# Xjh-UCAS/TAM-TR

Measured on AMD Instinct MI355X. Metric: images/sec fwd+bwd @640x640 bs=16/GPU, higher is better.
Workload: dtype bf16

## Files before the change

tam-tr_amd/csrc/dwconv.hip:

```cpp
#include "common.h"

namespace {

constexpr int TS = 16;
constexpr int DW_THREADS = TS * TS;
#ifndef DW_CB_BWD
#define DW_CB_BWD 16
#endif
constexpr int CB_FWD = 32, CB_BWD = DW_CB_BWD;

__device__ __forceinline__ float silu_f(float v) { return v / (1.f + __expf(-v)); }

template <typename T>
struct Vec16;
template <>
struct Vec16<float> {
  static constexpr int N = 4;
  static __device__ __forceinline__ void ld(const float* p, float (&o)[4]) {
    const float4 v = *reinterpret_cast<const float4*>(p);
    o[0] = v.x; o[1] = v.y; o[2] = v.z; o[3] = v.w;
  }
  static __device__ __forceinline__ void st(float* p, const float (&v)[4]) { *reinterpret_cast<float4*>(p) = make_float4(v[0], v[1], v[2], v[3]); }
};
template <>
struct Vec16<bf16_t> {
  static constexpr int N = 8;
  static __device__ __forceinline__ void ld(const bf16_t* p, float (&o)[8]) {
    const uint4 v = *reinterpret_cast<const uint4*>(p);
    const uint32_t w[4] = {v.x, v.y, v.z, v.w};
#pragma unroll
    for (int i = 0; i < 4; ++i) { o[2 * i] = __uint_as_float(w[i] << 16); o[2 * i + 1] = __uint_as_float(w[i] & 0xffff0000u); }
  }
  static __device__ __forceinline__ void st(bf16_t* p, const float (&v)[8]) {
    uint4 o;
    o.x = (uint32_t)f2bf(v[0]) | ((uint32_t)f2bf(v[1]) << 16); o.y = (uint32_t)f2bf(v[2]) | ((uint32_t)f2bf(v[3]) << 16);
    o.z = (uint32_t)f2bf(v[4]) | ((uint32_t)f2bf(v[5]) << 16); o.w = (uint32_t)f2bf(v[6]) | ((uint32_t)f2bf(v[7]) << 16);
    *reinterpret_cast<uint4*>(p) = o;
  }
};

__device__ __forceinline__ void plane_st(float* p, float v) { *p = v; }
__device__ __forceinline__ void plane_st(bf16_t* p, float v) { *p = f2bf(v); }
__device__ __forceinline__ float plane_ld(const float* p) { return *p; }
__device__ __forceinline__ float plane_ld(const bf16_t* p) { return bf2f(*p); }
__device__ __forceinline__ float4 plane_ld4(const float* p) { return *reinterpret_cast<const float4*>(p); }
__device__ __forceinline__ float4 plane_ld4(const bf16_t* p) {
  const uint2 v = *reinterpret_cast<const uint2*>(p);
  return make_float4(__uint_as_float(v.x << 16), __uint_as_float(v.x & 0xffff0000u), __uint_as_float(v.y << 16), __uint_as_float(v.y & 0xffff0000u));
}

template <typename T, int CB, int HALO, int PITCH>
__device__ __forceinline__ void stage_tile(const T* __restrict__ x, size_t xs, int b, int d0, int h0, int w0, int H, int W,
                                           float (*s)[TS + 2 * HALO][PITCH]) {
  constexpr int SIDE = TS + 2 * HALO, VN = Vec16<T>::N, GROUPS = CB / VN, TOTAL = SIDE * SIDE * GROUPS;
  constexpr int N_IT = (TOTAL + DW_THREADS - 1) / DW_THREADS;
  float v[N_IT][VN];
#pragma unroll
  for (int k = 0; k < N_IT; ++k) {
    const int it = min((int)threadIdx.x + k * DW_THREADS, TOTAL - 1);
    const int pix = it / GROUPS, gq = it - pix * GROUPS;
    const int py = pix / SIDE, px = pix - py * SIDE;
    const int h = min(max(h0 + py - HALO, 0), H - 1), w = min(max(w0 + px - HALO, 0), W - 1);
    Vec16<T>::ld(x + ((size_t)(b * H + h) * W + w) * xs + d0 + gq * VN, v[k]);
  }
#pragma unroll
  for (int k = 0; k < N_IT; ++k) {
    const int it = threadIdx.x + k * DW_THREADS;
    if (it < TOTAL) {
      const int pix = it / GROUPS, gq = it - pix * GROUPS;
      const int py = pix / SIDE, px = pix - py * SIDE;
      const int h = h0 + py - HALO, w = w0 + px - HALO;
      const float keep = (h >= 0 && h < H && w >= 0 && w < W) ? 1.f : 0.f;
#pragma unroll
      for (int j = 0; j < VN; ++j) s[gq * VN + j][py][px] = v[k][j] * keep;
    }
  }
}

template <typename T, typename PT>
__global__ __launch_bounds__(DW_THREADS) void dwconv_cross_fwd_kernel(const T* __restrict__ x, size_t xs, const float* __restrict__ wgt,
                                                                       const float* __restrict__ bias, PT* __restrict__ u2, int D,
                                                                       int H, int W, int tiles_w) {
  constexpr int CB = CB_FWD, SIDE = TS + 2, PITCH = SIDE + 1;
  __shared__ float s_in[CB][SIDE][PITCH];
  __shared__ float s_w[CB][10];
  const int th = blockIdx.x / tiles_w, tw = blockIdx.x - th * tiles_w;
  const int d0 = blockIdx.y * CB, b = blockIdx.z, h0 = th * TS, w0 = tw * TS;
  const size_t L = (size_t)H * W;
  for (int i = threadIdx.x; i < CB * 10; i += DW_THREADS) {
    const int c = i / 10, k = i - c * 10;
    s_w[c][k] = k < 9 ? wgt[(size_t)(d0 + c) * 9 + k] : (bias ? bias[d0 + c] : 0.f);
  }
  stage_tile<T, CB, 1, PITCH>(x, xs, b, d0, h0, w0, H, W, s_in);
  __syncthreads();
#pragma unroll
  for (int pass = 0; pass < 2; ++pass) {
    const int ty = pass == 0 ? threadIdx.x / TS : threadIdx.x % TS;
    const int tx = pass == 0 ? threadIdx.x % TS : threadIdx.x / TS;
    const int h = h0 + ty, w = w0 + tx;
    if (h >= H || w >= W) continue;
    PT* out = u2 + ((size_t)(b * 2 + pass) * D + d0) * L + (pass == 0 ? (size_t)h * W + w : (size_t)w * H + h);
    for (int c = 0; c < CB; ++c) {
      float acc = s_w[c][9];
#pragma unroll
      for (int ky = 0; ky < 3; ++ky)
#pragma unroll
        for (int kx = 0; kx < 3; ++kx) acc = fmaf(s_w[c][ky * 3 + kx], s_in[c][ty + ky][tx + kx], acc);
      plane_st(out + (size_t)c * L, silu_f(acc));
    }
  }
}

template <typename T, typename PT>
__global__ __launch_bounds__(DW_THREADS) void dwconv_cross_bwd_kernel(const PT* __restrict__ g2, const T* __restrict__ x, size_t xs,
                                                                       const float* __restrict__ wgt, const float* __restrict__ bias,
                                                                       T* __restrict__ gx, size_t gxs, float* __restrict__ ws, int D,
                                                                       int H, int W, int tiles_w, int tiles) {
  constexpr int CB = CB_BWD, XS = TS + 4, XP = XS + 1, GS = TS + 2, GP = GS + 1;
  __shared__ float s_x[CB][XS][XP];
  __shared__ float s_g[CB][GS][GP];
  __shared__ float s_w[CB][10];
  const int th = blockIdx.x / tiles_w, tw = blockIdx.x - th * tiles_w;
  const int d0 = blockIdx.y * CB, b = blockIdx.z, h0 = th * TS, w0 = tw * TS;
  const size_t L = (size_t)H * W;
  for (int i = threadIdx.x; i < CB * 10; i += DW_THREADS) {
    const int c = i / 10, k = i - c * 10;
    s_w[c][k] = k < 9 ? wgt[(size_t)(d0 + c) * 9 + k] : (bias ? bias[d0 + c] : 0.f);
  }
#ifndef DW_ABL_NOX
  stage_tile<T, CB, 2, XP>(x, xs, b, d0, h0, w0, H, W, s_x);
#endif
#ifndef DW_ABL_NOG
  if ((W & 3) == 0 && (H & 3) == 0) {
    constexpr int NV = 6, ITEMS_V = CB * GS * NV, N_ITV = (ITEMS_V + DW_THREADS - 1) / DW_THREADS;
#pragma unroll
    for (int plane = 0; plane < 2; ++plane) {
      const PT* gp = g2 + ((size_t)(b * 2 + plane) * D + d0) * L;
      float4 v[N_ITV];
#pragma unroll
      for (int k = 0; k < N_ITV; ++k) {
        const int it = min((int)threadIdx.x + k * DW_THREADS, ITEMS_V - 1);
        const int c = it / (GS * NV), r = it - c * (GS * NV), line = r / NV, q = r - line * NV;
        const int fixed = (plane == 0 ? h0 : w0) + line - 1, base = (plane == 0 ? w0 : h0) - 4 + 4 * q;
        const int nfix = plane == 0 ? H : W, nrun = plane == 0 ? W : H;
        const bool ok = fixed >= 0 && fixed < nfix && base >= 0 && base + 3 < nrun;
        const float4 t = plane_ld4(gp + (size_t)c * L + (size_t)min(max(fixed, 0), nfix - 1) * nrun + min(max(base, 0), nrun - 4));
        const float f = ok ? 1.f : 0.f;
        v[k] = make_float4(t.x * f, t.y * f, t.z * f, t.w * f);
      }
      if (plane == 1) __syncthreads();
#pragma unroll
      for (int k = 0; k < N_ITV; ++k) {
        const int it = threadIdx.x + k * DW_THREADS;
        if (it < ITEMS_V) {
          const int c = it / (GS * NV), r = it - c * (GS * NV), line = r / NV, q = r - line * NV;
          const float e[4] = {v[k].x, v[k].y, v[k].z, v[k].w};
#pragma unroll
          for (int j = 0; j < 4; ++j) {
            const int pos = 4 * q + j - 3;
            if (pos >= 0 && pos < GS) {
              if (plane == 0) s_g[c][line][pos] = e[j];
              else s_g[c][pos][line] += e[j];
            }
          }
        }
      }
    }
  } else {
  {
    constexpr int GB = 7, N_IT = ((CB * GS * GS + DW_THREADS - 1) / DW_THREADS + GB - 1) / GB * GB;
    const PT* gp = g2 + ((size_t)(b * 2 + 0) * D + d0) * L;
#pragma unroll 1
    for (int k0 = 0; k0 < N_IT; k0 += GB) {
      float v[GB];
#pragma unroll
      for (int k = 0; k < GB; ++k) {
        const int it = min((int)threadIdx.x + (k0 + k) * DW_THREADS, CB * GS * GS - 1);
        const int c = it / (GS * GS), r = it - c * (GS * GS), py = r / GS, px = r - py * GS;
        const int h = h0 + py - 1, w = w0 + px - 1;
        const bool ok = h >= 0 && h < H && w >= 0 && w < W;
        v[k] = plane_ld(gp + (size_t)c * L + (size_t)min(max(h, 0), H - 1) * W + min(max(w, 0), W - 1)) * (ok ? 1.f : 0.f);
      }
#pragma unroll
      for (int k = 0; k < GB; ++k) {
        const int it = threadIdx.x + (k0 + k) * DW_THREADS;
        if (it < CB * GS * GS) {
          const int c = it / (GS * GS), r = it - c * (GS * GS), py = r / GS, px = r - py * GS;
          s_g[c][py][px] = v[k];
        }
      }
    }
  }
  __syncthreads();
  {
    constexpr int GB = 7, N_IT = ((CB * GS * GS + DW_THREADS - 1) / DW_THREADS + GB - 1) / GB * GB;
    const PT* gp = g2 + ((size_t)(b * 2 + 1) * D + d0) * L;
#pragma unroll 1
    for (int k0 = 0; k0 < N_IT; k0 += GB) {
      float v[GB];
#pragma unroll
      for (int k = 0; k < GB; ++k) {
        const int it = min((int)threadIdx.x + (k0 + k) * DW_THREADS, CB * GS * GS - 1);
        const int c = it / (GS * GS), r = it - c * (GS * GS), px = r / GS, py = r - px * GS;
        const int h = h0 + py - 1, w = w0 + px - 1;
        const bool ok = h >= 0 && h < H && w >= 0 && w < W;
        v[k] = plane_ld(gp + (size_t)c * L + (size_t)min(max(w, 0), W - 1) * H + min(max(h, 0), H - 1)) * (ok ? 1.f : 0.f);
      }
#pragma unroll
      for (int k = 0; k < GB; ++k) {
        const int it = threadIdx.x + (k0 + k) * DW_THREADS;
        if (it < CB * GS * GS) {
          const int c = it / (GS * GS), r = it - c * (GS * GS), px = r / GS, py = r - px * GS;
          s_g[c][py][px] += v[k];
        }
      }
    }
  }
  }
#endif
  __syncthreads();
#ifndef DW_ABL_NOSILU
  {
    constexpr int TPC = DW_THREADS / CB;
    static_assert(DW_THREADS % CB == 0 && TPC <= WAVE && (TPC & (TPC - 1)) == 0, "a power-of-two lane group per channel");
    const int c = threadIdx.x / TPC, sub = threadIdx.x % TPC;
    float wk[9], dwk[10];
#pragma unroll
    for (int k9 = 0; k9 < 9; ++k9) { wk[k9] = s_w[c][k9]; dwk[k9] = 0.f; }
    dwk[9] = 0.f;
    const float bc = s_w[c][9];
    for (int r = sub; r < GS * GS; r += TPC) {
      const int px = r / GS, py = r - px * GS;
      const int h = h0 + py - 1, w = w0 + px - 1;
      float g = 0.f;
      if (h >= 0 && h < H && w >= 0 && w < W) {
        g = s_g[c][py][px];
        float xin[9], acc = bc;
#pragma unroll
        for (int ky = 0; ky < 3; ++ky)
#pragma unroll
          for (int kx = 0; kx < 3; ++kx) { xin[ky * 3 + kx] = s_x[c][py + ky][px + kx]; acc = fmaf(wk[ky * 3 + kx], xin[ky * 3 + kx], acc); }
        const float sg = 1.f / (1.f + __expf(-acc));
        g *= sg * (1.f + acc * (1.f - sg));
        if (py >= 1 && py <= TS && px >= 1 && px <= TS) {
#pragma unroll
          for (int k9 = 0; k9 < 9; ++k9) dwk[k9] = fmaf(g, xin[k9], dwk[k9]);
          dwk[9] += g;
        }
      }
      s_g[c][py][px] = g;
    }
#pragma unroll
    for (int k9 = 0; k9 < 10; ++k9) dwk[k9] = group_sum<TPC>(dwk[k9]);
    if (sub == 0) {
      float* o = ws + (((size_t)b * tiles + blockIdx.x) * D + d0 + c) * 10;
#pragma unroll
      for (int k9 = 0; k9 < 10; ++k9) o[k9] = dwk[k9];
    }
  }
#endif
  __syncthreads();
  const int ty = threadIdx.x / TS, tx = threadIdx.x % TS;
  float dxv[CB];
#pragma unroll
  for (int c = 0; c < CB; ++c) {
    float acc = 0.f;
#pragma unroll
    for (int ky = 0; ky < 3; ++ky)
#pragma unroll
      for (int kx = 0; kx < 3; ++kx) acc = fmaf(s_w[c][ky * 3 + kx], s_g[c][ty + 2 - ky][tx + 2 - kx], acc);
    dxv[c] = acc;
  }
  __syncthreads();
#pragma unroll
  for (int c = 0; c < CB; ++c) s_x[c][ty][tx] = dxv[c];
  __syncthreads();
  constexpr int VN = Vec16<T>::N, GROUPS = CB / VN;
  for (int it = threadIdx.x; it < TS * TS * GROUPS; it += DW_THREADS) {
    const int pix = it / GROUPS, gq = it - pix * GROUPS, py = pix / TS, px = pix - py * TS;
    const int h = h0 + py, w = w0 + px;
    if (h < H && w < W) {
      float v[VN];
#pragma unroll
      for (int j = 0; j < VN; ++j) v[j] = s_x[gq * VN + j][py][px];
      Vec16<T>::st(gx + ((size_t)(b * H + h) * W + w) * gxs + d0 + gq * VN, v);
    }
  }
}

}

static int dwconv_check(const void* a, const void* b, const void* c, int B, int D, int H, int W, long long xs, int dtype) {
  if (!a || !b || !c || B <= 0 || D <= 0 || H <= 0 || W <= 0 || xs < D) return TAMTR_EINVAL;
  if (dtype != TAMTR_F32 && dtype != TAMTR_BF16) return TAMTR_EINVAL;
  const int vn = dtype == TAMTR_F32 ? 4 : 8;
  if (D % CB_FWD || xs % vn || B > 65535 || D / CB_BWD > 65535) return TAMTR_EUNSUP;
  return TAMTR_OK;
}

extern "C" int tamtr_dwconv_silu_cross_fwd(const void* x, long long x_pixel_stride, const float* weight, const float* bias, void* u2,
                                           int B, int D, int H, int W, int dtype, int plane_dtype, void* stream) {
  const int rc = dwconv_check(x, weight, u2, B, D, H, W, x_pixel_stride, dtype);
  if (rc) return rc;
  if (plane_dtype != TAMTR_F32 && !(plane_dtype == TAMTR_BF16 && dtype == TAMTR_BF16)) return TAMTR_EINVAL;
  const int tiles_w = (W + TS - 1) / TS, tiles_h = (H + TS - 1) / TS;
  const dim3 grid(tiles_w * tiles_h, D / CB_FWD, B);
  hipStream_t s = (hipStream_t)stream;
  if (dtype == TAMTR_F32)
    hipLaunchKernelGGL((dwconv_cross_fwd_kernel<float, float>), grid, dim3(DW_THREADS), 0, s, (const float*)x, (size_t)x_pixel_stride, weight, bias,
                       (float*)u2, D, H, W, tiles_w);
  else if (plane_dtype == TAMTR_F32)
    hipLaunchKernelGGL((dwconv_cross_fwd_kernel<bf16_t, float>), grid, dim3(DW_THREADS), 0, s, (const bf16_t*)x, (size_t)x_pixel_stride, weight,
                       bias, (float*)u2, D, H, W, tiles_w);
  else
    hipLaunchKernelGGL((dwconv_cross_fwd_kernel<bf16_t, bf16_t>), grid, dim3(DW_THREADS), 0, s, (const bf16_t*)x, (size_t)x_pixel_stride, weight,
                       bias, (bf16_t*)u2, D, H, W, tiles_w);
  return tamtr_launch_status();
}

extern "C" int tamtr_dwconv_tiles(int H, int W) { return ((W + TS - 1) / TS) * ((H + TS - 1) / TS); }

extern "C" int tamtr_dwconv_silu_cross_bwd(const void* g2, const void* x, long long x_pixel_stride, const float* weight, const float* bias,
                                           void* gx, long long gx_pixel_stride, float* ws, int B, int D, int H, int W, int dtype,
                                           int plane_dtype, void* stream) {
  const int rc = dwconv_check(x, weight, g2, B, D, H, W, x_pixel_stride, dtype);
  if (rc) return rc;
  if (!gx || !ws || gx_pixel_stride < D || gx_pixel_stride % (dtype == TAMTR_F32 ? 4 : 8)) return TAMTR_EINVAL;
  if (plane_dtype != TAMTR_F32 && !(plane_dtype == TAMTR_BF16 && dtype == TAMTR_BF16)) return TAMTR_EINVAL;
  if ((uintptr_t)g2 % 16) return TAMTR_EUNSUP;
  const int tiles_w = (W + TS - 1) / TS, tiles_h = (H + TS - 1) / TS;
  const dim3 grid(tiles_w * tiles_h, D / CB_BWD, B);
  hipStream_t s = (hipStream_t)stream;
  if (dtype == TAMTR_F32)
    hipLaunchKernelGGL((dwconv_cross_bwd_kernel<float, float>), grid, dim3(DW_THREADS), 0, s, (const float*)g2, (const float*)x, (size_t)x_pixel_stride,
                       weight, bias, (float*)gx, (size_t)gx_pixel_stride, ws, D, H, W, tiles_w, tiles_w * tiles_h);
  else if (plane_dtype == TAMTR_F32)
    hipLaunchKernelGGL((dwconv_cross_bwd_kernel<bf16_t, float>), grid, dim3(DW_THREADS), 0, s, (const float*)g2, (const bf16_t*)x,
                       (size_t)x_pixel_stride, weight, bias, (bf16_t*)gx, (size_t)gx_pixel_stride, ws, D, H, W, tiles_w, tiles_w * tiles_h);
  else
    hipLaunchKernelGGL((dwconv_cross_bwd_kernel<bf16_t, bf16_t>), grid, dim3(DW_THREADS), 0, s, (const bf16_t*)g2, (const bf16_t*)x,
                       (size_t)x_pixel_stride, weight, bias, (bf16_t*)gx, (size_t)gx_pixel_stride, ws, D, H, W, tiles_w, tiles_w * tiles_h);
  return tamtr_launch_status();
}
```

Measured before the change: 210.1.

## Register-block dwconv backward into 2x2 patches with float2 shared-memory access

Reworks the depthwise-conv backward kernel so each lane processes 2x2 output patches per channel. It loads a 4x4 input window once with float2 shared-memory reads and reuses it for the SiLU recompute, the weight-gradient accumulation and the transposed dx convolution. Shared buffers are flattened with even pitches, so 8-byte vector loads stay aligned. The dx pass is now per-channel across lane groups instead of per-pixel across all channels, which removes a syncthreads and a register array of size CB. The risk is more shared-memory bank conflicts from the new pitches, plus higher register pressure from the unrolled patches.

```diff
diff --git a/tam-tr_amd/csrc/dwconv.hip b/tam-tr_amd/csrc/dwconv.hip
--- a/tam-tr_amd/csrc/dwconv.hip
+++ b/tam-tr_amd/csrc/dwconv.hip
@@ -49,9 +49,8 @@
   return make_float4(__uint_as_float(v.x << 16), __uint_as_float(v.x & 0xffff0000u), __uint_as_float(v.y << 16), __uint_as_float(v.y & 0xffff0000u));
 }
 
-template <typename T, int CB, int HALO, int PITCH>
-__device__ __forceinline__ void stage_tile(const T* __restrict__ x, size_t xs, int b, int d0, int h0, int w0, int H, int W,
-                                           float (*s)[TS + 2 * HALO][PITCH]) {
+template <typename T, int CB, int HALO, int PITCH, int CSTRIDE>
+__device__ __forceinline__ void stage_tile(const T* __restrict__ x, size_t xs, int b, int d0, int h0, int w0, int H, int W, float* s) {
   constexpr int SIDE = TS + 2 * HALO, VN = Vec16<T>::N, GROUPS = CB / VN, TOTAL = SIDE * SIDE * GROUPS;
   constexpr int N_IT = (TOTAL + DW_THREADS - 1) / DW_THREADS;
   float v[N_IT][VN];
@@ -72,7 +71,7 @@
       const int h = h0 + py - HALO, w = w0 + px - HALO;
       const float keep = (h >= 0 && h < H && w >= 0 && w < W) ? 1.f : 0.f;
 #pragma unroll
-      for (int j = 0; j < VN; ++j) s[gq * VN + j][py][px] = v[k][j] * keep;
+      for (int j = 0; j < VN; ++j) s[(gq * VN + j) * CSTRIDE + py * PITCH + px] = v[k][j] * keep;
     }
   }
 }
@@ -91,7 +90,7 @@
     const int c = i / 10, k = i - c * 10;
     s_w[c][k] = k < 9 ? wgt[(size_t)(d0 + c) * 9 + k] : (bias ? bias[d0 + c] : 0.f);
   }
-  stage_tile<T, CB, 1, PITCH>(x, xs, b, d0, h0, w0, H, W, s_in);
+  stage_tile<T, CB, 1, PITCH, SIDE * PITCH>(x, xs, b, d0, h0, w0, H, W, &s_in[0][0][0]);
   __syncthreads();
 #pragma unroll
   for (int pass = 0; pass < 2; ++pass) {
@@ -116,9 +115,10 @@
                                                                        const float* __restrict__ wgt, const float* __restrict__ bias,
                                                                        T* __restrict__ gx, size_t gxs, float* __restrict__ ws, int D,
                                                                        int H, int W, int tiles_w, int tiles) {
-  constexpr int CB = CB_BWD, XS = TS + 4, XP = XS + 1, GS = TS + 2, GP = GS + 1;
-  __shared__ float s_x[CB][XS][XP];
-  __shared__ float s_g[CB][GS][GP];
+  constexpr int CB = CB_BWD, XS = TS + 4, XP = 24, XC = XS * XP + 2, GS = TS + 2, GP = GS, GC = GS * GP;
+  static_assert(XP % 2 == 0 && XC % 4 == 2 && GP % 2 == 0 && GC % 2 == 0, "8-byte aligned patch rows");
+  __shared__ __attribute__((aligned(16))) float s_x[CB * XC];
+  __shared__ __attribute__((aligned(16))) float s_g[CB * GC];
   __shared__ float s_w[CB][10];
   const int th = blockIdx.x / tiles_w, tw = blockIdx.x - th * tiles_w;
   const int d0 = blockIdx.y * CB, b = blockIdx.z, h0 = th * TS, w0 = tw * TS;
@@ -128,7 +128,7 @@
     s_w[c][k] = k < 9 ? wgt[(size_t)(d0 + c) * 9 + k] : (bias ? bias[d0 + c] : 0.f);
   }
 #ifndef DW_ABL_NOX
-  stage_tile<T, CB, 2, XP>(x, xs, b, d0, h0, w0, H, W, s_x);
+  stage_tile<T, CB, 2, XP, XC>(x, xs, b, d0, h0, w0, H, W, s_x);
 #endif
 #ifndef DW_ABL_NOG
   if ((W & 3) == 0 && (H & 3) == 0) {
@@ -159,8 +159,8 @@
           for (int j = 0; j < 4; ++j) {
             const int pos = 4 * q + j - 3;
             if (pos >= 0 && pos < GS) {
-              if (plane == 0) s_g[c][line][pos] = e[j];
-              else s_g[c][pos][line] += e[j];
+              if (plane == 0) s_g[c * GC + line * GP + pos] = e[j];
+              else s_g[c * GC + pos * GP + line] += e[j];
             }
           }
         }
@@ -186,7 +186,7 @@
         const int it = threadIdx.x + (k0 + k) * DW_THREADS;
         if (it < CB * GS * GS) {
           const int c = it / (GS * GS), r = it - c * (GS * GS), py = r / GS, px = r - py * GS;
-          s_g[c][py][px] = v[k];
+          s_g[c * GC + py * GP + px] = v[k];
         }
       }
     }
@@ -211,44 +211,64 @@
         const int it = threadIdx.x + (k0 + k) * DW_THREADS;
         if (it < CB * GS * GS) {
           const int c = it / (GS * GS), r = it - c * (GS * GS), px = r / GS, py = r - px * GS;
-          s_g[c][py][px] += v[k];
-        }
-      }
-    }
-  }
-  }
-#endif
-  __syncthreads();
+          s_g[c * GC + py * GP + px] += v[k];
+        }
+      }
+    }
+  }
+  }
+#endif
+  __syncthreads();
+  constexpr int TPC = DW_THREADS / CB;
+  static_assert(DW_THREADS % CB == 0 && TPC <= WAVE && (TPC & (TPC - 1)) == 0, "a power-of-two lane group per channel");
+  static_assert(GS % 2 == 0 && TS % 2 == 0, "whole 2 x 2 patches");
+  const int c = threadIdx.x / TPC, sub = threadIdx.x % TPC;
+  float wk[9];
+#pragma unroll
+  for (int k9 = 0; k9 < 9; ++k9) wk[k9] = s_w[c][k9];
 #ifndef DW_ABL_NOSILU
   {
-    constexpr int TPC = DW_THREADS / CB;
-    static_assert(DW_THREADS % CB == 0 && TPC <= WAVE && (TPC & (TPC - 1)) == 0, "a power-of-two lane group per channel");
-    const int c = threadIdx.x / TPC, sub = threadIdx.x % TPC;
-    float wk[9], dwk[10];
-#pragma unroll
-    for (int k9 = 0; k9 < 9; ++k9) { wk[k9] = s_w[c][k9]; dwk[k9] = 0.f; }
-    dwk[9] = 0.f;
+    constexpr int PG = GS / 2;
+    float dwk[10];
+#pragma unroll
+    for (int k9 = 0; k9 < 10; ++k9) dwk[k9] = 0.f;
     const float bc = s_w[c][9];
-    for (int r = sub; r < GS * GS; r += TPC) {
-      const int px = r / GS, py = r - px * GS;
-      const int h = h0 + py - 1, w = w0 + px - 1;
-      float g = 0.f;
-      if (h >= 0 && h < H && w >= 0 && w < W) {
-        g = s_g[c][py][px];
-        float xin[9], acc = bc;
-#pragma unroll
-        for (int ky = 0; ky < 3; ++ky)
-#pragma unroll
-          for (int kx = 0; kx < 3; ++kx) { xin[ky * 3 + kx] = s_x[c][py + ky][px + kx]; acc = fmaf(wk[ky * 3 + kx], xin[ky * 3 + kx], acc); }
-        const float sg = 1.f / (1.f + __expf(-acc));
-        g *= sg * (1.f + acc * (1.f - sg));
-        if (py >= 1 && py <= TS && px >= 1 && px <= TS) {
-#pragma unroll
-          for (int k9 = 0; k9 < 9; ++k9) dwk[k9] = fmaf(g, xin[k9], dwk[k9]);
-          dwk[9] += g;
-        }
-      }
-      s_g[c][py][px] = g;
+    for (int q = sub; q < PG * PG; q += TPC) {
+      const int py = 2 * (q / PG), px = 2 * (q % PG);
+      float xin[4][4], g[2][2];
+#pragma unroll
+      for (int r = 0; r < 4; ++r) {
+        const float2 lo = *reinterpret_cast<const float2*>(&s_x[c * XC + (py + r) * XP + px]);
+        const float2 hi = *reinterpret_cast<const float2*>(&s_x[c * XC + (py + r) * XP + px + 2]);
+        xin[r][0] = lo.x; xin[r][1] = lo.y; xin[r][2] = hi.x; xin[r][3] = hi.y;
+      }
+#pragma unroll
+      for (int r = 0; r < 2; ++r) {
+        const float2 t = *reinterpret_cast<const float2*>(&s_g[c * GC + (py + r) * GP + px]);
+        g[r][0] = t.x; g[r][1] = t.y;
+      }
+#pragma unroll
+      for (int dy = 0; dy < 2; ++dy)
+#pragma unroll
+        for (int dx = 0; dx < 2; ++dx) {
+          float acc = bc;
+#pragma unroll
+          for (int ky = 0; ky < 3; ++ky)
+#pragma unroll
+            for (int kx = 0; kx < 3; ++kx) acc = fmaf(wk[ky * 3 + kx], xin[dy + ky][dx + kx], acc);
+          const float sg = 1.f / (1.f + __expf(-acc));
+          const float gv = g[dy][dx] * (sg * (1.f + acc * (1.f - sg)));
+          g[dy][dx] = gv;
+          const bool core = py + dy >= 1 && py + dy <= TS && px + dx >= 1 && px + dx <= TS;
+          const float gc = core ? gv : 0.f;
+#pragma unroll
+          for (int ky = 0; ky < 3; ++ky)
+#pragma unroll
+            for (int kx = 0; kx < 3; ++kx) dwk[ky * 3 + kx] = fmaf(gc, xin[dy + ky][dx + kx], dwk[ky * 3 + kx]);
+          dwk[9] += gc;
+        }
+#pragma unroll
+      for (int r = 0; r < 2; ++r) *reinterpret_cast<float2*>(&s_g[c * GC + (py + r) * GP + px]) = make_float2(g[r][0], g[r][1]);
     }
 #pragma unroll
     for (int k9 = 0; k9 < 10; ++k9) dwk[k9] = group_sum<TPC>(dwk[k9]);
@@ -260,20 +280,38 @@
   }
 #endif
   __syncthreads();
-  const int ty = threadIdx.x / TS, tx = threadIdx.x % TS;
-  float dxv[CB];
-#pragma unroll
-  for (int c = 0; c < CB; ++c) {
-    float acc = 0.f;
-#pragma unroll
-    for (int ky = 0; ky < 3; ++ky)
-#pragma unroll
-      for (int kx = 0; kx < 3; ++kx) acc = fmaf(s_w[c][ky * 3 + kx], s_g[c][ty + 2 - ky][tx + 2 - kx], acc);
-    dxv[c] = acc;
-  }
-  __syncthreads();
-#pragma unroll
-  for (int c = 0; c < CB; ++c) s_x[c][ty][tx] = dxv[c];
+#ifndef DW_ABL_NODX
+  {
+    constexpr int PC = TS / 2;
+    for (int q = sub; q < PC * PC; q += TPC) {
+      const int py = 2 * (q / PC), px = 2 * (q % PC);
+      float gin[4][4];
+#pragma unroll
+      for (int r = 0; r < 4; ++r) {
+        const float2 lo = *reinterpret_cast<const float2*>(&s_g[c * GC + (py + r) * GP + px]);
+        const float2 hi = *reinterpret_cast<const float2*>(&s_g[c * GC + (py + r) * GP + px + 2]);
+        gin[r][0] = lo.x; gin[r][1] = lo.y; gin[r][2] = hi.x; gin[r][3] = hi.y;
+      }
+#pragma unroll
+      for (int dy = 0; dy < 2; ++dy) {
+        float o[2];
+#pragma unroll
+        for (int dx = 0; dx < 2; ++dx) {
+          float acc = 0.f;
+#pragma unroll
+          for (int ky = 0; ky < 3; ++ky)
+#pragma unroll
+            for (int kx = 0; kx < 3; ++kx) acc = fmaf(wk[ky * 3 + kx], gin[dy + 2 - ky][dx + 2 - kx], acc);
+          o[dx] = acc;
+        }
+        *reinterpret_cast<float2*>(&s_x[c * XC + (py + dy) * XP + px]) = make_float2(o[0], o[1]);
+      }
+    }
+  }
+#endif
+#ifdef DW_ABL_NOST
+  return;
+#endif
   __syncthreads();
   constexpr int VN = Vec16<T>::N, GROUPS = CB / VN;
   for (int it = threadIdx.x; it < TS * TS * GROUPS; it += DW_THREADS) {
@@ -282,7 +320,7 @@
     if (h < H && w < W) {
       float v[VN];
 #pragma unroll
-      for (int j = 0; j < VN; ++j) v[j] = s_x[gq * VN + j][py][px];
+      for (int j = 0; j < VN; ++j) v[j] = s_x[(gq * VN + j) * XC + py * XP + px];
       Vec16<T>::st(gx + ((size_t)(b * H + h) * W + w) * gxs + d0 + gq * VN, v);
     }
   }
```

Result: no change. 210.7 (median of 6 runs) (+0.3%).
